# maetyu-d/audio-suite

Hardware: AMD Instinct MI355X
Metric: Msamples/sec rendered (microsound full pipe, 384 kHz->48 kHz) at 1/2/4/8 GPUs (higher is better)
Workload: dtype fp32; 1 GPU; C3: 384 kHz out, unfold x100 (30 MHz design SR), stretch x2, Poisson 18/s, 1 s, 16k-tap IR request (8192 cap), ER 320 taps, stereo; presets_per_gpu=1024, frames_per_gpu_step=393216000, sub_batches_per_gpu=3, parallelism=preset-sharded x1, streams_per_gpu=3, stream_gate=2,4, enqueue=threads

## Files before the change

audio-suite_amd/csrc/ctx.h:

```cpp
#pragma once
#include <atomic>
#include <cstdlib>
#include <cstring>
#include <map>
#include <memory>
#include <mutex>
#include <string>
#include <vector>

#include "dev_own.h"
#include "host_pool.h"

namespace {

std::mutex g_gate_mu;

struct Staging {
    struct Item { void** slot; const void* src; size_t bytes; };
    struct Slot { PinnedBuf host; Event done; bool armed = false; };
    Slot slot[2];
    int cur = 0;
    DevBuf<char> arena;
    std::vector<Item> items;
    template <class T> void add(T** dst, const T* src, size_t bytes) {
        items.push_back(Item{reinterpret_cast<void**>(dst), src, bytes});
    }
    hipError_t flush(hipStream_t s) {
        Slot& sl = slot[cur];
        hipError_t e = hipSuccess;
        if (!sl.done) e = sl.done.create(hipEventDisableTiming);
        if (e == hipSuccess && sl.armed) e = hipEventSynchronize(sl.done);
        std::vector<size_t> at(items.size());
        size_t total = 0;
        for (size_t i = 0; i < items.size(); ++i) {
            at[i] = total;
            total += (items[i].bytes + 255) & ~size_t(255);
        }
        total = std::max<size_t>(total, 256);
        if (e == hipSuccess && total > sl.host.cap) e = sl.host.alloc(total + total / 4 + 4096);
        if (e == hipSuccess && total > arena.cap) e = arena.alloc(total + total / 4 + 4096);
        if (e == hipSuccess) {
            constexpr size_t PIECE = size_t(1) << 20;
            std::vector<std::pair<size_t, size_t>> pieces;
// ... 17 lines not shown
    }
};

template <class T> struct Slice { T* p = nullptr; };

template <class P, class S>
struct PlanStoreT {
    std::vector<P> host;
    std::vector<DevBuf<S>> allocs;
    std::map<int, int> by_n;
    bool dirty = false;
    DevBuf<P> dev;
};
using PlanStore = PlanStoreT<RealPlan, float>;
using Plan64Store = PlanStoreT<Real64Plan, double>;

struct Switches {
    bool device_plan = false;
    bool fir4 = true;
    bool fir4c = true;
    bool fir8 = true;
    int fir64 = 1;
    int fir64_cap = FIR64_CAP;
    int fir8p = 1;
    bool fir8q = true;
    int fir8p_cus = 0;
    bool ola_fir = true;
    double ola_fir_density = 1.25;
    int h_early = 2;
    bool er_dev = true;
    int so_row = 0, so_col = 0;
    bool gen_share = true;
    bool spec_share = true;

    static Switches from_env() {
        Switches w;
        if (const char* e = getenv("MSGPU_DEVICE_PLAN")) w.device_plan = e[0] == '1';
        if (const char* e = getenv("MSGPU_FIR4")) w.fir4 = e[0] != '0';
        if (const char* e = getenv("MSGPU_FIR4C")) w.fir4c = e[0] != '0';
        if (const char* e = getenv("MSGPU_FIR8")) w.fir8 = e[0] != '0';
        if (const char* e = getenv("MSGPU_FIR64")) w.fir64 = atoi(e);
        if (const char* e = getenv("MSGPU_FIR64_CAP")) w.fir64_cap = std::max(1, std::min(FIR64_CAP, atoi(e)));
        if (const char* e = getenv("MSGPU_FIR8P")) w.fir8p = atoi(e);
        if (const char* e = getenv("MSGPU_FIR8Q")) w.fir8q = e[0] != '0';
        if (const char* e = getenv("MSGPU_FIR8P_CUS")) w.fir8p_cus = std::max(0, atoi(e));
        if (const char* e = getenv("MSGPU_OLA_FIR")) w.ola_fir = e[0] != '0';
        if (const char* e = getenv("MSGPU_OLA_FIR_DENSITY")) w.ola_fir_density = atof(e);
        if (const char* e = getenv("MSGPU_H_EARLY")) w.h_early = atoi(e);
        if (const char* e = getenv("MSGPU_ER_DEV")) w.er_dev = e[0] != '0';
        if (const char* e = getenv("MSGPU_SO_ROW")) w.so_row = atoi(e);
        if (const char* e = getenv("MSGPU_SO_COL")) w.so_col = atoi(e);
        if (const char* e = getenv("MSGPU_GEN_SHARE")) w.gen_share = e[0] != '0';
        if (const char* e = getenv("MSGPU_SPEC_SHARE")) w.spec_share = e[0] != '0';
        if (!w.gen_share) w.spec_share = false;        return w;
    }
};

struct Gate {
    msg_ctx* peer = nullptr;
    std::vector<msg_ctx*> gated_by;
    int wait = -1, rec = -1;
    Event ev;
    std::atomic<bool> armed{false};
};

struct Prof {
    bool on = false;
    int every = 1;
    int64_t n = 0;
    bool batch = false;
    Event ev[2][12];
    int cur = 0;
    bool pending[2] = {false, false};
    bool pending_fir[2] = {false, false};
    bool pending_h_early[2] = {false, false};
    double stage_sum[10] = {0};
    int64_t stage_cnt = 0;
    double host_sum[8] = {0};
    double ola_fir_sum = 0.0;
    double gen_events_sum = 0.0, gen_grains_sum = 0.0;
    double spec_runs_sum = 0.0;
    int64_t host_cnt = 0;

    hipError_t create_events() {
        for (auto& set : ev)
            for (Event& e : set)
                if (const hipError_t err = e.create()) return err;
// ... 171 lines not shown
```

audio-suite_amd/csrc/host_abi.inc:

```

int64_t msg_sizeof(int32_t which) {
    switch (which) {
        case 0: return (int64_t)sizeof(msg_preset);
        case 1: return (int64_t)sizeof(msg_event);
        case 2: return (int64_t)sizeof(msg_plan_info);
        case 3: return (int64_t)sizeof(msg_digest_rec);
        case 4: return (int64_t)sizeof(msg_loudness_rec);
        case 5: return (int64_t)sizeof(msg_truepeak_rec);
        case 6: return (int64_t)sizeof(msg_pcm_rec);
        case 7: return (int64_t)sizeof(msg_limit_rec);
        case 8: return (int64_t)sizeof(msg_lrange_rec);
        default: return -1;
    }
}

int msg_plan_host(const msg_preset* preset, const double* bp_bank, const double* ir_frag, int64_t ir_frag_len,
                  msg_plan_info* info, msg_event* events, int32_t max_events,
                  int32_t* er_off, double* er_gain) {
    (void)ir_frag;
    if (!preset || !info) return fail(nullptr, MSG_E_ARG, "null argument");
    for (int l = 0; l < 4; ++l)
        if (preset->n_bp[l] < 0 || (preset->n_bp[l] > 0 && (!bp_bank || preset->bp_off[l] < 0)))
            return fail(nullptr, MSG_E_ARG, "bad breakpoint lane");
    msg_plan_info sz;
// ... 225 lines not shown
            for (;;) {
                if (id == 0) {
                    for (;;) {
                        const double xx = -nprng::ZIG_NOR_INV_R * log1p(-nprng::next_double(g));
                        const double yy = -log1p(-nprng::next_double(g));
                        c += 2;
                        if (yy + yy > xx * xx) { v = ((ra >> 8) & 1) ? -(nprng::ZIG_NOR_R + xx) : nprng::ZIG_NOR_R + xx; break; }
                    }
                    break;
                }
                const double u = nprng::next_double(g);
                c += 1;
                if (((zig_fi_double[id - 1] - zig_fi_double[id]) * u + zig_fi_double[id]) < exp(-0.5 * xv * xv)) { v = xv; break; }
                uint64_t r = nprng::next_u64(g);
                c += 1;
                id = (int)(r & 0xff); r >>= 8;
                const int sign = (int)(r & 1);
                ra = (r >> 1) & 0x000fffffffffffffULL;
                xv = (double)ra * zig_wi_double[id];
                if (sign) xv = -xv;
                if (ra < zig_ki_double[id]) { v = xv; break; }
            }
            if (produced < n) out[produced] = v;
            ++produced;
            local = q + c;
        }
        do {
            for (int l = 0; l < 64; ++l) st[l] = j64.a * st[l] + g0.inc * j64.s;
            local -= 64;
        } while (local >= 64);
    }
    return MSG_OK;
}
```

audio-suite_amd/csrc/kernels_core.h:

```cpp
#pragma once
#include "rt.h"
#include "ola.h"
#include <type_traits>

__global__ void k_plan_sizes(const msg_preset* __restrict__ presets, int n_presets,
                             const double* __restrict__ bp, const int64_t* __restrict__ frag_len, nprng::Zig z,
                             msg_plan_info* __restrict__ info) {
    const int p = blockIdx.x * blockDim.x + threadIdx.x;
    if (p >= n_presets) return;
    msg_plan_info inf;
    msgplan::plan_sizes(presets[p], bp, z, frag_len[p], inf);
    info[p] = inf;
}

__global__ void k_plan_events(const msg_preset* __restrict__ presets, int n_presets,
                              const double* __restrict__ bp, const int64_t* __restrict__ frag_len, nprng::Zig z,
                              const int32_t* __restrict__ slot_base, const int32_t* __restrict__ tap_base,
                              msg_event* __restrict__ events, int32_t* __restrict__ er_off,
                              double* __restrict__ er_gain, msg_plan_info* __restrict__ info) {
    const int p = blockIdx.x * blockDim.x + threadIdx.x;
    if (p >= n_presets) return;
    msg_plan_info inf;
    const msg_preset& pr = presets[p];
    const bool er = (pr.flags & MSG_F_ER_CLOUD) != 0;
    msgplan::plan_events(pr, bp, z, frag_len[p], p, inf, events + slot_base[p],
                         er ? er_off + tap_base[p] : nullptr, er ? er_gain + tap_base[p] : nullptr);
    info[p] = inf;
}

#ifndef MSG_GEN_G
#define MSG_GEN_G 8
#endif
constexpr int GEN_G = MSG_GEN_G;
struct JumpTab {
    nprng::u128 a[GEN_T]; nprng::u128 s[GEN_T]; nprng::u128 a64, s64, aG, sG;
    uint2 kw[256]; float fif[256];
};

template <int G>
MSG_DEV int gen_walk(const uint64_t (&F)[G], const int (&consumed)[G], int local, uint32_t& vb, int& cnt) {
    cnt = 0;
    vb = 0;
#pragma unroll
    for (int g = 0; g < G; ++g) {
        if (local >= 64) { local -= 64; continue; }
        uint64_t valid = ~0ULL << local;
        uint64_t S = ~F[g] & valid;
        int pos = 64;
        while (S) {
            const int q = __builtin_ctzll(S);
            const int end = q + __builtin_amdgcn_readlane(consumed[g], q);
            const uint64_t after_q = ~((2ULL << q) - 1);
            const uint64_t before_end = end >= 64 ? ~0ULL : ((1ULL << end) - 1);
            valid &= ~(after_q & before_end);
            if (end >= 64) { pos = end; break; }
            S &= ~0ULL << end;
        }
        if (__builtin_amdgcn_inverse_ballot_w64(valid)) vb |= 1u << g;
        cnt += __popcll(valid);
        local = pos - 64;
    }
    return local;
}

MSG_DEV double slow_normal(nprng::u128 st, nprng::u128 inc, uint64_t rabs, int idx, double x,
                           const nprng::Zig& z, const uint64_t* ki, const double* wi, const float* fif,
                           int& consumed) {
    nprng::Pcg64 g;
    g.state = st; g.inc = inc; g.has_u32 = 0; g.u32 = 0;
// ... 62 lines not shown
    const float bv = h2 - hi;
    lo += (hi - (h2 - bv)) + (fl - bv);
    hi = h2;
    const float a = 2.0f * hi;
    const float sn = sinpif(a), cs = cospif(a);
    const float d = 6.2831853071795865f * lo;
    return make_float2(fmaf(d, cs, sn), fmaf(-d, sn, cs));
}
MSG_DEV float gen_basic_sample(const GenBasicConst& c, int j, float nrm) {
    float x;
    const float jf = (float)j;
    if (c.mode == MSG_GEN_RESONANT) {
        const float ph = ring_phase(jf, c.fa, c.fb);
        x = 0.9f * __builtin_amdgcn_sinf(ph) * __builtin_amdgcn_exp2f(fmaxf(jf * c.k_ring, -126.f)) +
            0.25f * nrm * __builtin_amdgcn_exp2f(fmaxf(jf * c.k_exc, -126.f));
    } else if (c.mode == MSG_GEN_GAUSSIAN_CLICK) {
        const float u = jf * c.inv_sigma;
        x = expf(-0.5f * (u * u)) * (nrm * 0.12f + 1.0f);
    } else if (c.mode == MSG_GEN_NOISE_BURST || c.mode == MSG_GEN_SKEWED) {
        return nrm;
    } else {
        x = nrm * 0.1f;
    }
    if (j < c.fade) x *= jf * c.inv_fade;
    if (j >= c.n - c.fade) x *= (float)(j - (c.n - c.fade)) * -c.inv_fade + 1.0f;
    return x;
}
MSG_DEV float gen_fade(const GenBasicConst& c, int j, float x) {
    if (j < c.fade) x *= (float)j * c.inv_fade;
    if (j >= c.n - c.fade) x *= (float)(j - (c.n - c.fade)) * -c.inv_fade + 1.0f;
    return x;
}

template <bool RAW64>
__global__ void __launch_bounds__(GEN_T)
k_gen_normal(const msg_preset* __restrict__ presets, const msg_event* __restrict__ events,
             const PresetRt* __restrict__ rt, const int32_t* __restrict__ ev_list, int n_list,
             nprng::Zig z, const JumpTab* __restrict__ jt, float* __restrict__ pool,
             double* __restrict__ pool64, const int64_t* __restrict__ off64) {
    __shared__ uint64_t s_ki[256];
    __shared__ double s_wi[256];
    __shared__ uint2 s_kw[256];
    __shared__ float s_fif[256];
    __shared__ float4 s_rot[128];
    __shared__ float4 s_base[64];
    const int li = blockIdx.x;
    if (li >= n_list) return;
    const int lane = (int)(threadIdx.x & (GEN_T - 1));
    for (int i = (int)threadIdx.x; i < 256; i += GEN_T) {
        s_ki[i] = z.ki[i];
        s_wi[i] = z.wi[i];
        s_kw[i] = jt->kw[i];
        s_fif[i] = jt->fif[i];
    }
    const msg_event& e = events[ev_list[li]];
    const msg_preset& pr = presets[e.preset];
    const PresetRt& r = rt[e.preset];
    const int n = e.n;
    float* out = pool + r.pool_base + e.pool_off;
    double* out64 = RAW64 ? pool64 + off64[li] : nullptr;

    GenBasicConst c;
    c.mode = pr.gen_mode == MSG_GEN_FALLBACK ? MSG_GEN_NOISE_BURST : pr.gen_mode;
    c.n = n;
    c.fade = (int)(0.01 * n) > 8 ? (int)(0.01 * n) : 8;
    c.inv_fade = (float)(1.0 / (double)c.fade);
    const double inv_sr = 1.0 / (double)e.gen_sr;
    const double f_over_sr = fmax(10.0, pr.ring_hz) * inv_sr;
    c.fa = (float)f_over_sr;
    c.fb = (float)(f_over_sr - (double)c.fa);
    const double log2e = 1.4426950408889634;
    c.k_ring = (float)(-inv_sr / fmax(1e-6, pr.ring_decay_ms / 1000.0) * log2e);
    c.k_exc = (float)(-inv_sr / fmax(1e-6, (pr.micro_ms / 1000.0) * 0.15) * log2e);
    const int sigma = (int)(0.0025 * n) > 1 ? (int)(0.0025 * n) : 1;
    c.inv_sigma = (float)(1.0 / (double)sigma);
    int q0 = -64;
    if (!RAW64 && c.mode == MSG_GEN_RESONANT) {
        for (int i = (int)threadIdx.x; i < 128; i += GEN_T) {
            const float rf = (float)i;
            const float2 sc = ring_sincos(rf, c.fa, c.fb);
            s_rot[i] = make_float4(sc.y, sc.x, 0.9f * __builtin_amdgcn_exp2f(rf * c.k_ring),
                                   0.25f * __builtin_amdgcn_exp2f(rf * c.k_exc));
        }
    }

    const nprng::Pcg64 g0 = nprng::default_rng((uint64_t)(pr.seed + e.index));
    const nprng::u128 inc = g0.inc;
    const nprng::u128 a64 = jt->a64;
    const nprng::u128 c64 = inc * jt->s64;

    constexpr int G = GEN_G;
    nprng::u128 st[G];
    st[0] = jt->a[lane] * g0.state + inc * jt->s[lane];
#pragma unroll
    for (int g = 1; g < G; ++g) st[g] = a64 * st[g - 1] + c64;
    const nprng::u128 aG = jt->aG;
    const nprng::u128 cG = inc * jt->sG;
    __syncthreads();

    int produced = 0;
    int local = 0;
    while (produced < n) {
        using XT = typename std::conditional<RAW64, double, float>::type;
        uint64_t rabs[G], F[G];
        int idx[G], consumed[G];
        (void)rabs; (void)idx;
        XT x[G];
        unsigned slow = 0;
#pragma unroll
        for (int g = 0; g < G; ++g) {
            consumed[g] = 1;
            bool fast;
            if constexpr (RAW64) {
                const uint64_t raw = nprng::xsl_rr(st[g]);
                const int id = (int)(raw & 0xff);
                const uint64_t rr = raw >> 8;
                rabs[g] = (rr >> 1) & 0x000fffffffffffffULL;
                idx[g] = id | (int)((rr & 1) << 8);
                x[g] = (double)rabs[g] * s_wi[id];
                if (rr & 1) x[g] = -x[g];
                fast = rabs[g] < s_ki[id];
            } else {
                const uint64_t hi = (uint64_t)(st[g] >> 64), lo = (uint64_t)st[g];
                const uint32_t rot = (uint32_t)(hi >> 58);
                uint32_t xl = (uint32_t)(hi ^ lo), xh = (uint32_t)((hi ^ lo) >> 32);
                if (rot & 32) { const uint32_t tmp = xl; xl = xh; xh = tmp; }
                const uint32_t olo = __builtin_amdgcn_alignbit(xh, xl, rot);
                const uint32_t ohi = __builtin_amdgcn_alignbit(xl, xh, rot);
                const uint32_t r32 = __builtin_amdgcn_alignbit(ohi, olo, 29);
                const int id = (int)(olo & 0xff);
                const uint2 kw = s_kw[id];
                const float xf = (float)r32 * __uint_as_float(kw.y);
                x[g] = (olo & 0x100) ? -xf : xf;
                fast = r32 < kw.x;
            }
            F[g] = __ballot(fast);
            if (!fast) slow |= 1u << g;
        }
        while (slow) {
            const int gs = __builtin_ctz(slow);
            slow &= slow - 1;
            nprng::u128 s0 = st[0];
#pragma unroll
            for (int g = 1; g < G; ++g)
                if (gs == g) s0 = st[g];
            const uint64_t raw = nprng::xsl_rr(s0);
            const int id = (int)(raw & 0xff);
            const uint64_t ra = (raw >> 9) & 0x000fffffffffffffULL;
            if (!RAW64 && ra < s_ki[id]) continue;
            double xv = (double)ra * s_wi[id];
            if ((raw >> 8) & 1) xv = -xv;
            int cn = 1;
            const double v = slow_normal(s0, inc, ra, id, xv, z, s_ki, s_wi, s_fif, cn);
#pragma unroll
            for (int g = 0; g < G; ++g)
                if (gs == g) { x[g] = (XT)v; consumed[g] = cn; }
        }
        uint32_t vb;
        int cnt;
        int pc = produced;
        local = gen_walk<G>(F, consumed, local, vb, cnt);
        produced += cnt;
        const bool reson = !RAW64 && c.mode == MSG_GEN_RESONANT;
#pragma unroll
        for (int g = 0; g < G; ++g) {
            const uint64_t valid = __ballot((vb >> g) & 1u);
            if (pc >= n || !valid) continue;
            if constexpr (RAW64) {
                if ((valid >> lane) & 1) {
                    const int j = pc + __popcll(valid & ((1ULL << lane) - 1));
                    if (j < n) out64[j] = x[g];
                }
            } else {
                const int rk = (int)__builtin_amdgcn_mbcnt_hi((uint32_t)(valid >> 32),
                                                              __builtin_amdgcn_mbcnt_lo((uint32_t)valid, 0u));
                const bool vl = __builtin_amdgcn_inverse_ballot_w64(valid);
                const int room = n - pc;
                float* __restrict__ ob = out + pc;
                if (reson) {
                    const int q = pc >> 6, d = pc & 63;
                    if (q - q0 >= 64) {
                        q0 = q;
                        const float jb = (float)(64 * (q0 + lane));
                        const float2 sc = ring_sincos(jb, c.fa, c.fb);
                        __syncthreads();
                        s_base[lane] = make_float4(sc.x, sc.y, __builtin_amdgcn_exp2f(fmaxf(jb * c.k_ring, -126.f)),
                                                   __builtin_amdgcn_exp2f(fmaxf(jb * c.k_exc, -126.f)));
                        __syncthreads();
                    }
                    const float4 u = s_base[q - q0];
                    const bool edge = pc < c.fade || pc + 64 > c.n - c.fade;
                    if (vl && rk < room) {
                        const float4 tb = s_rot[rk + d];
                        float v = fmaf(u.x, tb.x, u.y * tb.y) * (u.z * tb.z) + x[g] * (u.w * tb.w);
                        if (edge) v = gen_fade(c, pc + rk, v);
                        ob[rk] = v;
                    }
                } else if (vl && rk < room) {
                    ob[rk] = gen_basic_sample(c, pc + rk, (float)x[g]);
                }
            }
            pc += __popcll(valid);
        }
#pragma unroll
        for (int g = 0; g < G; ++g) st[g] = aG * st[g] + cG;
    }
}

constexpr int ER_T = 256;

MSG_DEV double er_uniform(nprng::Pcg64& g, double lo, double hi) {
    return __dadd_rn(lo, __dmul_rn(hi - lo, nprng::next_double(g)));
}

__global__ void __launch_bounds__(ER_T)
k_er_gains(const msg_preset* __restrict__ presets, const PresetRt* __restrict__ rt, int n_presets,
           const int32_t* __restrict__ er_key, const int32_t* __restrict__ er_first,
           const int32_t* __restrict__ er_cnt, double* __restrict__ g_tap, double* __restrict__ er_gain) {
    const int p = blockIdx.x;
    if (p >= n_presets) return;
    const msg_preset& pr = presets[p];
    if (!(pr.flags & MSG_F_ER_CLOUD)) return;
    const PresetRt& r = rt[p];
// ... 109 lines not shown
```

audio-suite_amd/csrc/msgpu.hip:

```cpp
#include <hip/hip_runtime.h>
#include <algorithm>
#include <cmath>
#include <cstdio>
#include <cstring>
#include <deque>
#include <map>
#include <sched.h>
#include <atomic>
#include <chrono>
#include <condition_variable>
#include <functional>
#include <memory>
#include <mutex>
#include <optional>
#include <string>
#include <thread>
#include <vector>

#include "msg_common.h"
#include "ziggurat_tables.h"
#include "nprng.h"
#include "plan.h"
#include "fftplan.h"
#include "fft_lds.h"
// ... 295 lines not shown
}

template <class T>
static int sf_upload(msg_ctx* ctx, hipStream_t s, const std::vector<PresetRt>& prt, const std::vector<int2>& jobs,
                     const int64_t* irjobs, size_t n_irjobs, DevBuf<T>& taps_dev, const T* taps, int64_t M) {
    HIPCHK(ctx, ctx->sf_prt.ensure(prt.size()));
    HIPCHK(ctx, ctx->sf_jobs.ensure(jobs.size()));
    HIPCHK(ctx, taps_dev.ensure((size_t)M));
    HIPCHK(ctx, ctx->sf_irjobs.ensure(n_irjobs));
    HIPCHK(ctx, hipMemcpyAsync(ctx->sf_prt.p, prt.data(), sizeof(PresetRt) * prt.size(), hipMemcpyHostToDevice, s));
    HIPCHK(ctx, hipMemcpyAsync(ctx->sf_jobs.p, jobs.data(), sizeof(int2) * jobs.size(), hipMemcpyHostToDevice, s));
    HIPCHK(ctx, hipMemcpyAsync(taps_dev.p, taps, sizeof(T) * (size_t)M, hipMemcpyHostToDevice, s));
    HIPCHK(ctx, hipMemcpyAsync(ctx->sf_irjobs.p, irjobs, sizeof(int64_t) * n_irjobs, hipMemcpyHostToDevice, s));
    return MSG_OK;
}

extern "C" {

int msg_abi_version(void) { return MSG_ABI_VERSION; }

int msg_host_threads(void) { return HostPool::get().threads(); }

const char* msg_last_error(msg_ctx* ctx) { return ctx ? ctx->err.c_str() : g_err.c_str(); }

msg_ctx* msg_create(int device_ordinal) {
    int ndev = 0;
    hipError_t e = hipGetDeviceCount(&ndev);
    if (e != hipSuccess || ndev <= 0) { g_err = "no HIP device available"; return nullptr; }
    if (device_ordinal < 0 || device_ordinal >= ndev) { g_err = "bad device ordinal"; return nullptr; }
    if (hipSetDevice(device_ordinal) != hipSuccess) { g_err = "hipSetDevice failed"; return nullptr; }
    std::unique_ptr<msg_ctx> ctx(new msg_ctx());
    ctx->device = device_ordinal;
    ctx->sw = Switches::from_env();
    auto up = [](auto& dst, const auto* src, size_t n) { return dst.upload(src, n) == hipSuccess; };
    auto up2 = [](DevBuf<float2>& dst, bool ok, const std::vector<float>& tab) {
        return ok && dst.upload(reinterpret_cast<const float2*>(tab.data()), tab.size() / 2) == hipSuccess;
    };
    if (!up(ctx->d_ki, zig_ki_double, 256) || !up(ctx->d_wi, zig_wi_double, 256) ||
        !up(ctx->d_fi, zig_fi_double, 256) || !up(ctx->d_ke, zig_ke_double, 256) ||
        !up(ctx->d_we, zig_we_double, 256) || !up(ctx->d_fe, zig_fe_double, 256)) {
        g_err = "uploading ziggurat tables failed";
        return nullptr;
    }
    ctx->dzig = nprng::Zig{ctx->d_ki.p, ctx->d_wi.p, ctx->d_fi.p, ctx->d_ke.p, ctx->d_we.p, ctx->d_fe.p};
    JumpTab jt;
    for (int l = 0; l < GEN_T; ++l) {
        const nprng::Jump j = nprng::jump_of((uint64_t)l + 1);
        jt.a[l] = j.a; jt.s[l] = j.s;
    }
    const nprng::Jump j64 = nprng::jump_of(GEN_T);
    jt.a64 = j64.a; jt.s64 = j64.s;
    const nprng::Jump jG = nprng::jump_of((uint64_t)GEN_T * GEN_G);
    jt.aG = jG.a; jt.sG = jG.s;
    for (int i = 0; i < 256; ++i) {
        const float w = (float)(zig_wi_double[i] * 1048576.0);
        uint32_t wb;
        memcpy(&wb, &w, 4);
        jt.kw[i] = make_uint2((uint32_t)(zig_ki_double[i] >> 20), wb);
        jt.fif[i] = (float)zig_fi_double[i];
    }
    if (!up(ctx->d_jump, &jt, 1)) { g_err = "uploading jump table failed"; return nullptr; }
    std::vector<float> tab;
    for (int i = 0; i < 5; ++i)
        if (!up2(ctx->d_fir2tab[i], fir2_tables_host(1024 << i, tab), tab)) {
            g_err = "uploading FIR twiddle tables failed";
            return nullptr;
        }
    if (!up2(ctx->d_fir4tab, fir4_tables_host(16384, tab), tab)) {
        g_err = "uploading FIR4 twiddle tables failed";
        return nullptr;
    }
    for (int i = 0; i < SPEC_CT_PLANS; ++i)
        if (!up2(ctx->d_spec_ct_tab[i], spectral_ct_tables(i, tab), tab)) {
            g_err = "uploading spectral twiddle tables failed";
            return nullptr;
        }
    if (!up2(ctx->d_spec3_tab, spec3_tables(tab), tab)) {
        g_err = "uploading spectral twiddle tables failed";
        return nullptr;
    }
    {
        float tp_tab[TP_TAB_N];
        tp_table(tp_tab);
        if (!up(ctx->d_tp_tab, tp_tab, (size_t)TP_TAB_N)) { g_err = "uploading the true-peak taps failed"; return nullptr; }
    }
    int cu = 0;
// ... 391 lines not shown
```

audio-suite_amd/csrc/render_stages.h:

```cpp
#pragma once

static int stage_check(msg_ctx* ctx, Batch& b) {
    for (int p = 0; p < b.P; ++p) {
        for (int l = 0; l < 4; ++l) {
            const int32_t nb = b.presets[p].n_bp[l], ob = b.presets[p].bp_off[l];
            if (nb < 0 || (nb > 0 && (!b.bp_bank || ob < 0 || (int64_t)ob + nb > b.bp_pairs)))
                return fail(ctx, MSG_E_ARG, "preset " + std::to_string(p) + ": breakpoint lane outside the bank");
        }
        const int ic = b.presets[p].ir_conv;
        if (ic >= b.n_irs || (ic >= 0 && !b.irs)) return fail(ctx, MSG_E_ARG, "bad IR index");
    }
    return MSG_OK;
}

static int plan_bases(msg_ctx* ctx, Batch& b) {
    b.nslots = b.ntaps = 0;
    int64_t frames = 0;
    for (int p = 0; p < b.P; ++p) {
        b.slot_base[p] = (int32_t)b.nslots;
        b.tap_base[p] = (int32_t)b.ntaps;
        b.nslots += b.info[p].n_slots;
        if (b.presets[p].flags & MSG_F_ER_CLOUD) b.ntaps += std::max(1, b.presets[p].er_taps);
        if (b.info[p].out_n > MSG_MAX_FRAMES) return fail(ctx, MSG_E_UNSUPPORTED, "output longer than 2^31 - 2^20 frames");
        frames += b.info[p].out_n;
// ... 752 lines not shown
static int enqueue_h_spectra(msg_ctx* ctx, Batch& b) {
    const Batch::Fir& F = b.fir;
    hipStream_t s = b.s;
    const double* erg = er_gains(ctx, b);
    if (b.er_dev && b.ntaps > 0) {
        hipLaunchKernelGGL(k_er_gains, dim3((unsigned)b.P), dim3(ER_T), 0, s, ctx->presets.p, ctx->prt.p, b.P,
                           ctx->er_key.p, ctx->er_first.p, ctx->er_cnt.p, ctx->er_tap_d.p, ctx->er_gain_d.p);
        HIPCHK(ctx, hipGetLastError());
    }
    if (F.htiles > 0)
        HIPCHK(ctx, launch_h_build((unsigned)F.htiles, s, ctx->prt.p, ctx->h_tile_begin.p, b.P, ctx->er_off.p,
                                   erg, ctx->irbank.p, ctx->hscratch.p));
    if (!F.ir8.jobs.empty())
        HIPCHK(ctx, launch_fir8_spec64((unsigned)(F.ir8.jobs.size() / 4), s, ctx->ir8_jobs.p, ctx->d_fir4tab.p,
                                       ctx->irbank.p, ctx->hspec.p));
    if (!F.hpart_jobs.empty())
        HIPCHK(ctx, launch_fir4_hpart(16384, (unsigned)F.hpart_jobs.size(), s, ctx->prt.p, ctx->hpart_jobs.p,
                                      ctx->d_fir4tab.p, ctx->hscratch.p, ctx->hspec.p));
    if (!F.ir8.er_list.empty())
        HIPCHK(ctx, launch_fir8_hconv((unsigned)F.ir8.er_list.size(), s, ctx->prt.p, ctx->fir8_list.p, ctx->d_fir4tab.p,
                                      ctx->er_off.p, erg, ctx->hspec.p));
    if (!F.ir4.jobs.empty())
        HIPCHK(ctx, launch_fir4_irspec((unsigned)(F.ir4.jobs.size() / 4), s, ctx->ir4_jobs.p, ctx->d_fir4tab.p,
                                       ctx->irbank.p, ctx->hspec.p));
    if (!F.ir4.er_list.empty())
        HIPCHK(ctx, launch_fir4_hconv((unsigned)F.ir4.er_list.size(), s, ctx->prt.p, ctx->fir4c_list.p, ctx->d_fir4tab.p,
                                      ctx->er_off.p, erg, ctx->hspec.p));
    if (F.hblocks_gen > 0)
        HIPCHK(ctx, launch_fir_h((unsigned)F.hblocks, F.lds, s, ctx->prt.p, ctx->h_begin.p, b.P,
                                 ctx->fir_plans.dev.p, ctx->fir_plan_of.p, ctx->hscratch.p, ctx->hspec.p));
    return MSG_OK;
}

static int enqueue_generate(msg_ctx* ctx, Batch& b) {
    const std::vector<int32_t>& gen = b.f32.gen_list;
    const std::vector<int32_t>& gen64 = b.g64.gen_list;
    if (!gen.empty())
        hipLaunchKernelGGL(k_gen_normal<false>, dim3((unsigned)gen.size()), dim3(GEN_T), 0, b.s,
                           ctx->presets.p, ctx->events.p, ctx->prt.p, ctx->gen_list.p, (int)gen.size(),
                           ctx->dzig, ctx->d_jump.p, ctx->micro.p, (double*)nullptr, (const int64_t*)nullptr);
    HIPCHK(ctx, hipGetLastError());
    if (!gen64.empty())
        hipLaunchKernelGGL(k_gen_normal<true>, dim3((unsigned)gen64.size()), dim3(GEN_T), 0, b.s,
                           ctx->presets.p, ctx->events.p, ctx->prt.p, ctx->gen64_list.p, (int)gen64.size(),
                           ctx->dzig, ctx->d_jump.p, ctx->micro.p, ctx->micro64.p, (const int64_t*)ctx->gen64_off.p);
    HIPCHK(ctx, hipGetLastError());
    return MSG_OK;
}

static int enqueue_spectral(msg_ctx* ctx, Batch& b) {
    const Batch::F32& F = b.f32;
    const Batch::G64& G = b.g64;
    hipStream_t s = b.s;
    if (!F.spec3.empty())
        HIPCHK(ctx, launch_spec3((unsigned)F.spec3.size(), s, ctx->events.p, ctx->ert.p, ctx->prt.p, ctx->d_spec3_tab.p,
                                 ctx->spec3_list.p, (int)F.spec3.size(), ctx->micro.p, ctx->grain.p));
    for (int i = 0; i < SPEC_CT_PLANS; ++i)
        if (F.ct_off[i + 1] > F.ct_off[i])
            HIPCHK(ctx, launch_spectral_ct(i, (unsigned)(F.ct_off[i + 1] - F.ct_off[i]), s, ctx->events.p, ctx->ert.p,
                                           ctx->prt.p, ctx->d_spec_ct_tab[i].p, ctx->spec_ct_list.p + F.ct_off[i],
                                           F.ct_off[i + 1] - F.ct_off[i], ctx->micro.p, ctx->grain.p));
    if (!F.spec_small.empty())
        HIPCHK(ctx, launch_spectral(false, (unsigned)F.spec_small.size(), F.small_lds, s, ctx->presets.p,
                                    ctx->events.p, ctx->ert.p, ctx->prt.p, ctx->grain_plans.dev.p, ctx->spec_small.p,
                                    (int)F.spec_small.size(), ctx->micro.p, ctx->grain.p));
    if (!F.spec_big.empty())
        HIPCHK(ctx, launch_spectral(true, (unsigned)F.spec_big.size(), F.big_lds, s, ctx->presets.p,
                                    ctx->events.p, ctx->ert.p, ctx->prt.p, ctx->grain_plans.dev.p, ctx->spec_big.p,
                                    (int)F.spec_big.size(), ctx->micro.p, ctx->grain.p));
    if (!G.lds.empty())
        HIPCHK(ctx, launch_grain64(nullptr, (unsigned)G.lds.size(), G.cap * 16, s, ctx->presets.p, ctx->ev64.p,
                                   ctx->prt.p, ctx->plans64.dev.p, ctx->g64_list.p, (int)G.lds.size(),
                                   ctx->irbank.p, ctx->imgbank.p, ctx->dzig, ctx->micro64.p, ctx->grain64.p,
                                   ctx->save64.p, ctx->grain.p));
    if (!G.glb.empty())
        HIPCHK(ctx, launch_grain64(&G.gg, G.g_grid, 0, s, ctx->presets.p, ctx->ev64.p, ctx->prt.p, ctx->plans64.dev.p,
                                   ctx->g64_list.p + G.lds.size(), (int)G.glb.size(), ctx->irbank.p,
                                   ctx->imgbank.p, ctx->dzig, ctx->micro64.p, ctx->grain64.p, ctx->save64.p,
// ... 184 lines not shown
```

audio-suite_amd/msgpu/_lib.py:

```python
from __future__ import annotations

import ctypes as C
import os
import threading

HERE = os.path.dirname(os.path.abspath(__file__))
LIB_PATH = os.environ.get("MSGPU_LIB") or os.path.join(HERE, "libmsgpu.so")
ABI_VERSION = 2

MSG_OK, MSG_E_VALUE, MSG_E_UNSUPPORTED, MSG_E_DEVICE, MSG_E_ARG = 0, 1, 2, 3, 4

SPEC_ROUTES = ("copy", "small", "big", "ct37500", "ct30000", "ct2400", "ct1920", "ct1500", "ct480", "spec3", "f64")

GEN_MODE = {"Gaussian click": 0, "Dust impulses": 1, "Noise burst": 2, "Skewed transient": 3,
            "Resonant strike": 4, "Crackle / corona": 5, "Stick–slip friction": 6,
            "Micro-chaos": 7, "Wavelet atoms": 8, "IR fragment": 9, "Image scanline": 10}
GEN_FALLBACK = 11
PROCESS = {"Single": 0, "Poisson": 1, "Clustered": 2, "Hawkes": 3}
PROC_NONE = 4
F_STEREO, F_BANDLIMIT, F_PARTIAL_LOCK, F_NL_WARP, F_CEP_WARP, F_GRAIN_OFFSET = (1 << i for i in range(6))
F_RES_BANK, F_WAVEGUIDE, F_EVENT_FEEDBACK, F_IMPRINT, F_ER_CLOUD, F_SPACE_IR, F_MULTIBAND = \
    (1 << i for i in range(6, 13))


# ... 116 lines not shown
    "msg_loudness": (C.c_int, [C.c_void_p, C.c_void_p, C.c_int32, C.POINTER(C.c_int64), C.POINTER(C.c_int64), C.c_int32,
                               C.c_int32, C.c_void_p, C.c_void_p]),
    "msg_loudness_range": (C.c_int, [C.c_void_p, C.c_void_p, C.c_int32, C.POINTER(C.c_int64), C.POINTER(C.c_int64),
                                     C.c_int32, C.c_int32, C.c_void_p, C.c_void_p, C.c_void_p, C.POINTER(C.c_int64),
                                     C.c_void_p]),
    "msg_lrange_hops_host": (C.c_int, [C.c_void_p, C.c_int64, C.c_int64, C.c_void_p]),
    "msg_loudness_range_host": (C.c_int, [C.c_void_p, C.c_int32, C.c_int64, C.c_int32, C.c_void_p, C.c_void_p]),
    "msg_loudness_gain": (C.c_int, [C.c_void_p, C.c_void_p, C.c_int32, C.POINTER(C.c_int64), C.POINTER(C.c_int64),
                                    C.c_int32, C.c_void_p, C.c_double, C.c_double, C.c_void_p]),
    "msg_loudness_host": (C.c_int, [C.c_void_p, C.c_int32, C.c_int64, C.c_int32, C.c_void_p]),
    "msg_truepeak": (C.c_int, [C.c_void_p, C.c_void_p, C.c_int32, C.POINTER(C.c_int64), C.POINTER(C.c_int64), C.c_int32,
                               C.c_int32, C.c_void_p, C.c_void_p]),
    "msg_truepeak_gain": (C.c_int, [C.c_void_p, C.c_void_p, C.c_int32, C.POINTER(C.c_int64), C.POINTER(C.c_int64),
                                    C.c_int32, C.c_void_p, C.c_void_p, C.c_double, C.c_double, C.c_double, C.c_void_p]),
    "msg_truepeak_host": (C.c_int, [C.c_void_p, C.c_int32, C.c_int64, C.c_int32, C.c_void_p]),
    "msg_quantize": (C.c_int, [C.c_void_p, C.c_void_p, C.c_int32, C.POINTER(C.c_int64), C.POINTER(C.c_int64), C.c_int32,
                               C.c_int32, C.c_int32, C.c_uint64, C.POINTER(C.c_uint64), C.c_void_p,
                               C.POINTER(C.c_int64), C.c_void_p, C.c_void_p]),
    "msg_quantize_host": (C.c_int, [C.c_void_p, C.c_int32, C.c_int64, C.c_int32, C.c_int32, C.c_uint64, C.c_uint64,
                                    C.c_void_p, C.c_void_p]),
    "msg_quantize_shaped": (C.c_int, [C.c_void_p, C.c_void_p, C.c_int32, C.POINTER(C.c_int64), C.POINTER(C.c_int64),
                                      C.c_int32, C.c_int32, C.c_int32, C.c_int32, C.c_uint64, C.POINTER(C.c_uint64),
                                      C.c_void_p, C.POINTER(C.c_int64), C.c_void_p, C.c_void_p]),
    "msg_quantize_shaped_host": (C.c_int, [C.c_void_p, C.c_int32, C.c_int64, C.c_int32, C.c_int32, C.c_int32, C.c_uint64,
                                           C.c_uint64, C.c_void_p, C.c_void_p]),
    "msg_limit": (C.c_int, [C.c_void_p, C.c_void_p, C.c_int32, C.POINTER(C.c_int64), C.POINTER(C.c_int64), C.c_int32,
                            C.c_int32, C.c_double, C.c_int32, C.c_void_p, C.c_void_p, C.c_void_p]),
    "msg_limit_host": (C.c_int, [C.c_void_p, C.c_int32, C.c_int64, C.c_int32, C.c_double, C.c_int32, C.c_void_p]),
    "msg_rng_raw": (C.c_int, [C.c_uint64, C.POINTER(C.c_uint64), C.c_int64]),
    "msg_rng_normal": (C.c_int, [C.c_uint64, C.POINTER(C.c_double), C.c_int64]),
    "msg_rng_exponential": (C.c_int, [C.c_uint64, C.POINTER(C.c_double), C.c_int64]),
    "msg_rng_integers": (C.c_int, [C.c_uint64, C.c_int64, C.c_int64, C.POINTER(C.c_int64), C.c_int64]),
    "msg_rng_normal_chunked": (C.c_int, [C.c_uint64, C.POINTER(C.c_double), C.c_int64]),
}
EXPORTS = tuple(_PROTOS)

_lib = None
_lock = threading.Lock()


def lib() -> C.CDLL:
    global _lib
    with _lock:
        if _lib is None:
            if not os.path.exists(LIB_PATH):
                raise RuntimeError(f"libmsgpu not built: {LIB_PATH} is missing "
                                   "(run `python -c 'import __graft_entry__ as g; g.build()'`)")
            if os.environ.get("MSGPU_HOST_ONLY") != "1":
                try:
                    import torch
                except ImportError:
                    pass
            L = C.CDLL(LIB_PATH)
            for name, (res, args) in _PROTOS.items():
                f = getattr(L, name)
                f.restype = res
                f.argtypes = args
            if L.msg_abi_version() != ABI_VERSION:
                raise RuntimeError("libmsgpu ABI version mismatch")
            for which, st in enumerate((MsgPreset, MsgEvent, MsgPlanInfo, MsgDigestRec, MsgLoudnessRec,
                                        MsgTruePeakRec, MsgPcmRec, MsgLimitRec, MsgLRangeRec)):
                if L.msg_sizeof(which) != C.sizeof(st):
                    raise RuntimeError(f"libmsgpu struct {st.__name__} size mismatch: "
                                       f"{L.msg_sizeof(which)} != {C.sizeof(st)}")
            _lib = L
    return _lib
# ... 12 lines not shown
```

include/msgpu.h:

```cpp
#ifndef MSGPU_H
#define MSGPU_H

#include <stddef.h>
#include <stdint.h>

#ifdef __cplusplus
extern "C" {
#endif

#define MSG_ABI_VERSION 2

enum msg_gen_mode {
    MSG_GEN_GAUSSIAN_CLICK = 0, MSG_GEN_DUST = 1, MSG_GEN_NOISE_BURST = 2,
    MSG_GEN_SKEWED = 3, MSG_GEN_RESONANT = 4, MSG_GEN_CRACKLE = 5,
    MSG_GEN_STICK_SLIP = 6, MSG_GEN_MICRO_CHAOS = 7, MSG_GEN_WAVELET = 8,
    MSG_GEN_IR_FRAGMENT = 9, MSG_GEN_IMAGE = 10,
    MSG_GEN_FALLBACK = 11
};
enum msg_process { MSG_PROC_SINGLE = 0, MSG_PROC_POISSON = 1, MSG_PROC_CLUSTERED = 2,
                   MSG_PROC_HAWKES = 3, MSG_PROC_NONE = 4 };
enum msg_flag {
    MSG_F_STEREO = 1u << 0, MSG_F_BANDLIMIT = 1u << 1, MSG_F_PARTIAL_LOCK = 1u << 2,
    MSG_F_NL_WARP = 1u << 3, MSG_F_CEP_WARP = 1u << 4, MSG_F_GRAIN_OFFSET = 1u << 5,
    MSG_F_RES_BANK = 1u << 6, MSG_F_WAVEGUIDE = 1u << 7, MSG_F_EVENT_FEEDBACK = 1u << 8,
// ... 151 lines not shown
    int32_t q_min, q_max;
    int32_t bits, dither;
} msg_pcm_rec;
int msg_quantize(msg_ctx* ctx, const float* x_dev, int32_t channels, const int64_t* offsets, const int64_t* n,
                 int32_t n_signals, int32_t bits, int32_t dither, uint64_t seed, const uint64_t* keys,
                 void* out_dev, const int64_t* out_byte_off, msg_pcm_rec* rec_dev, void* stream);
int msg_quantize_host(const float* x, int32_t channels, int64_t n, int32_t bits, int32_t dither, uint64_t seed,
                      uint64_t key, void* out, msg_pcm_rec* rec);

enum msg_shape { MSG_SHAPE_E3 = 1, MSG_SHAPE_LIPSHITZ5 = 2, MSG_SHAPE_F9 = 3 };
int msg_quantize_shaped(msg_ctx* ctx, const float* x_dev, int32_t channels, const int64_t* offsets, const int64_t* n,
                        int32_t n_signals, int32_t bits, int32_t dither, int32_t shape, uint64_t seed,
                        const uint64_t* keys, void* out_dev, const int64_t* out_byte_off, msg_pcm_rec* rec_dev,
                        void* stream);
int msg_quantize_shaped_host(const float* x, int32_t channels, int64_t n, int32_t bits, int32_t dither, int32_t shape,
                             uint64_t seed, uint64_t key, void* out, msg_pcm_rec* rec);

typedef struct msg_limit_rec {
    double min_gain, reduction_db;
    int64_t limited_frames;
    int32_t lookahead, state;
} msg_limit_rec;
int msg_limit(msg_ctx* ctx, float* x_dev, int32_t channels, const int64_t* offsets, const int64_t* n,
              int32_t n_signals, int32_t sr, double ceiling_tp, int32_t lookahead_frames,
              const msg_truepeak_rec* tp_rec_dev, msg_limit_rec* rec_dev, void* stream);
int msg_limit_host(float* x, int32_t channels, int64_t n, int32_t sr, double ceiling_tp,
                   int32_t lookahead_frames, msg_limit_rec* rec);

int msg_rng_raw(uint64_t seed, uint64_t* out, int64_t n);
int msg_rng_normal(uint64_t seed, double* out, int64_t n);
int msg_rng_exponential(uint64_t seed, double* out, int64_t n);
int msg_rng_integers(uint64_t seed, int64_t low, int64_t high, int64_t* out, int64_t n);
int msg_rng_normal_chunked(uint64_t seed, double* out, int64_t n);

#ifdef __cplusplus
}
#endif
#endif
```

Measured before the change: 88580 Msamples/s.

## Split each event's normal generation across K cooperating waves

The normal-noise generator kernel now launches K waves per event. Each wave jumps the PCG stream to its own 512-draw group, classifies its draws independently, and then the waves stitch their ziggurat carry-over offsets in order through shared memory, re-walking only when a group's carry is nonzero. A host rule picks K from list length, event length and CU count so that short lists of long events fill the GPU, and MSGPU_GEN_K can override it. The cost is extra block barriers per round and larger blocks. Host reference functions are added to check the wave-split ordering.

```diff
diff --git a/audio-suite_amd/csrc/ctx.h b/audio-suite_amd/csrc/ctx.h
--- a/audio-suite_amd/csrc/ctx.h
+++ b/audio-suite_amd/csrc/ctx.h
@@ -9,6 +9,7 @@
 #include <vector>
 
 #include "dev_own.h"
+#include "gen_waves.h"
 #include "host_pool.h"
 
 namespace {
@@ -92,6 +93,7 @@
     int so_row = 0, so_col = 0;
     bool gen_share = true;
     bool spec_share = true;
+    int gen_k = 0;
 
     static Switches from_env() {
         Switches w;
@@ -112,7 +114,9 @@
         if (const char* e = getenv("MSGPU_SO_COL")) w.so_col = atoi(e);
         if (const char* e = getenv("MSGPU_GEN_SHARE")) w.gen_share = e[0] != '0';
         if (const char* e = getenv("MSGPU_SPEC_SHARE")) w.spec_share = e[0] != '0';
-        if (!w.gen_share) w.spec_share = false;        return w;
+        if (const char* e = getenv("MSGPU_GEN_K")) w.gen_k = (e[0] >= '0' && e[0] <= '9') ? atoi(e) : -1;
+        if (!w.gen_share) w.spec_share = false;
+        return w;
     }
 };
 
diff --git a/audio-suite_amd/csrc/gen_waves.h b/audio-suite_amd/csrc/gen_waves.h
--- /dev/null
+++ b/audio-suite_amd/csrc/gen_waves.h
@@ -0,0 +1,26 @@
+#pragma once
+#include <cstdint>
+
+namespace genwaves {
+
+constexpr int KMAX = 16;
+constexpr int GROUP = 512;
+constexpr int WAVES_PER_CU = 16;
+constexpr int LONG_LIST_PER_CU = 8;
+constexpr int SHARED_K = 4;
+constexpr int SMALL_LIST_PER_CU_INV = 4;
+
+inline bool valid_k(int k) { return k == 1 || k == 2 || k == 4 || k == 8 || k == 16; }
+
+inline int gen_waves(int64_t list_len, int64_t n_max, int n_cu) {
+    if (list_len <= 0 || n_max <= GROUP || n_cu <= 0) return 1;
+    if (list_len >= (int64_t)LONG_LIST_PER_CU * n_cu) return 1;
+    const int64_t groups = (n_max + GROUP - 1) / GROUP;
+    const int64_t room = (int64_t)WAVES_PER_CU * n_cu / list_len;
+    const int kmax = list_len * SMALL_LIST_PER_CU_INV <= n_cu ? KMAX : SHARED_K;
+    int k = 1;
+    while (2 * k <= kmax && 2 * k <= groups && 2 * k <= room) k *= 2;
+    return k;
+}
+
+}
diff --git a/audio-suite_amd/csrc/host_abi.inc b/audio-suite_amd/csrc/host_abi.inc
--- a/audio-suite_amd/csrc/host_abi.inc
+++ b/audio-suite_amd/csrc/host_abi.inc
@@ -281,3 +281,123 @@
     }
     return MSG_OK;
 }
+
+namespace {
+constexpr int KW_GROUP = 512;
+struct KwGroup {
+    double x[KW_GROUP];
+    int consumed[KW_GROUP];
+    int cnt = 0, over = 0;
+    int first = 0;
+};
+void kw_classify(nprng::u128 st, nprng::u128 inc, const nprng::Jump& j1, KwGroup& G) {
+    for (int l = 0; l < KW_GROUP; ++l) {
+        st = j1.a * st + inc * j1.s;
+        const uint64_t raw = nprng::xsl_rr(st);
+        int id = (int)(raw & 0xff);
+        const uint64_t rr = raw >> 8;
+        uint64_t ra = (rr >> 1) & 0x000fffffffffffffULL;
+        double xv = (double)ra * zig_wi_double[id];
+        if (rr & 1) xv = -xv;
+        G.x[l] = xv;
+        G.consumed[l] = 1;
+        if (ra < zig_ki_double[id]) continue;
+        nprng::Pcg64 g;
+        g.state = st; g.inc = inc; g.has_u32 = 0; g.u32 = 0;
+        int c = 1;
+        double v = 0.0;
+        for (;;) {
+            if (id == 0) {
+                for (;;) {
+                    const double xx = -nprng::ZIG_NOR_INV_R * log1p(-nprng::next_double(g));
+                    const double yy = -log1p(-nprng::next_double(g));
+                    c += 2;
+                    if (yy + yy > xx * xx) { v = ((ra >> 8) & 1) ? -(nprng::ZIG_NOR_R + xx) : nprng::ZIG_NOR_R + xx; break; }
+                }
+                break;
+            }
+            const double u = nprng::next_double(g);
+            c += 1;
+            if (((zig_fi_double[id - 1] - zig_fi_double[id]) * u + zig_fi_double[id]) < exp(-0.5 * xv * xv)) { v = xv; break; }
+            uint64_t r = nprng::next_u64(g);
+            c += 1;
+            id = (int)(r & 0xff); r >>= 8;
+            const int sign = (int)(r & 1);
+            ra = (r >> 1) & 0x000fffffffffffffULL;
+            xv = (double)ra * zig_wi_double[id];
+            if (sign) xv = -xv;
+            if (ra < zig_ki_double[id]) { v = xv; break; }
+        }
+        G.x[l] = v;
+        G.consumed[l] = c;
+    }
+}
+void kw_walk(KwGroup& G, int local) {
+    G.first = local;
+    G.cnt = 0;
+    int p = local;
+    while (p < KW_GROUP) { p += G.consumed[p]; ++G.cnt; }
+    G.over = p - KW_GROUP;
+}
+void kw_emit(const KwGroup& G, int64_t pw, double* out, int64_t n) {
+    int64_t j = pw;
+    for (int p = G.first; p < KW_GROUP && j < n; p += G.consumed[p]) out[j++] = G.x[p];
+}
+}
+
+int msg_rng_normal_kwaves(uint64_t seed, int32_t K, double* out, int64_t n, int64_t* rewalks) {
+    if (!(K == 1 || K == 2 || K == 4 || K == 8 || K == 16)) return fail(nullptr, MSG_E_VALUE, "K must be 1, 2, 4, 8 or 16");
+    if (n < 0 || (n > 0 && !out)) return fail(nullptr, MSG_E_VALUE, "bad output");
+    const nprng::Pcg64 g0 = nprng::default_rng(seed);
+    const nprng::Jump j1 = nprng::jump_of(1);
+    const nprng::Jump jR = nprng::jump_of((uint64_t)KW_GROUP * (uint64_t)K);
+    std::vector<KwGroup> grp((size_t)K);
+    std::vector<nprng::u128> st((size_t)K);
+    for (int w = 0; w < K; ++w) st[w] = nprng::apply_jump(nprng::jump_of((uint64_t)KW_GROUP * (uint64_t)w), g0.state, g0.inc);
+    int64_t produced = 0, rw = 0;
+    int local = 0;
+    while (produced < n) {
+        for (int w = 0; w < K; ++w) {
+            kw_classify(st[w], g0.inc, j1, grp[w]);
+            kw_walk(grp[w], 0);
+        }
+        int lin = local;
+        for (int j = 0; j < K; ++j) {
+            if (lin != 0) {
+                if (lin >= KW_GROUP) { grp[j].first = KW_GROUP; grp[j].cnt = 0; grp[j].over = lin - KW_GROUP; }
+                else kw_walk(grp[j], lin);
+                ++rw;
+            }
+            kw_emit(grp[j], produced, out, n);
+            produced += grp[j].cnt;
+            lin = grp[j].over;
+        }
+        local = lin;
+        for (int w = 0; w < K; ++w) st[w] = jR.a * st[w] + g0.inc * jR.s;
+    }
+    if (rewalks) *rewalks = rw;
+    return MSG_OK;
+}
+
+int64_t msg_rng_normal_carries(uint64_t seed, int64_t n, int32_t* carry, int64_t max_groups) {
+    if (n < 0 || max_groups < 0 || (max_groups > 0 && !carry)) return -1;
+    const nprng::Pcg64 g0 = nprng::default_rng(seed);
+    const nprng::Jump j1 = nprng::jump_of(1);
+    const nprng::Jump jG = nprng::jump_of((uint64_t)KW_GROUP);
+    std::vector<KwGroup> Gv(1);
+    KwGroup* const G = Gv.data();
+    nprng::u128 st = g0.state;
+    int64_t produced = 0, groups = 0;
+    int local = 0;
+    while (produced < n) {
+        if (groups < max_groups) carry[groups] = local;
+        kw_classify(st, g0.inc, j1, *G);
+        if (local >= KW_GROUP) { G->cnt = 0; G->over = local - KW_GROUP; }
+        else kw_walk(*G, local);
+        produced += G->cnt;
+        local = G->over;
+        st = jG.a * st + g0.inc * jG.s;
+        ++groups;
+    }
+    return groups;
+}
diff --git a/audio-suite_amd/csrc/kernels_core.h b/audio-suite_amd/csrc/kernels_core.h
--- a/audio-suite_amd/csrc/kernels_core.h
+++ b/audio-suite_amd/csrc/kernels_core.h
@@ -32,9 +32,13 @@
 #define MSG_GEN_G 8
 #endif
 constexpr int GEN_G = MSG_GEN_G;
+constexpr int GEN_KMAX = 16;
+MSG_HD constexpr int gen_k_log2(int k) { return k <= 1 ? 0 : 1 + gen_k_log2(k / 2); }
 struct JumpTab {
     nprng::u128 a[GEN_T]; nprng::u128 s[GEN_T]; nprng::u128 a64, s64, aG, sG;
     uint2 kw[256]; float fif[256];
+    nprng::u128 aW[GEN_KMAX], sW[GEN_KMAX];
+    nprng::u128 aR[4], sR[4];
 };
 
 template <int G>
@@ -163,8 +167,8 @@
     return x;
 }
 
-template <bool RAW64>
-__global__ void __launch_bounds__(GEN_T)
+template <bool RAW64, int K>
+__global__ void __launch_bounds__(GEN_T * K)
 k_gen_normal(const msg_preset* __restrict__ presets, const msg_event* __restrict__ events,
              const PresetRt* __restrict__ rt, const int32_t* __restrict__ ev_list, int n_list,
              nprng::Zig z, const JumpTab* __restrict__ jt, float* __restrict__ pool,
@@ -174,11 +178,17 @@
     __shared__ uint2 s_kw[256];
     __shared__ float s_fif[256];
     __shared__ float4 s_rot[128];
-    __shared__ float4 s_base[64];
+    __shared__ float4 s_base[K * 64];
+    __shared__ int2 s_carry[2][K];
+    static_assert(K == 1 || K == 2 || K == 4 || K == 8 || K == GEN_KMAX, "waves per event");
+    (void)s_carry;
     const int li = blockIdx.x;
     if (li >= n_list) return;
     const int lane = (int)(threadIdx.x & (GEN_T - 1));
-    for (int i = (int)threadIdx.x; i < 256; i += GEN_T) {
+    int wv = 0;
+    if constexpr (K > 1) wv = __builtin_amdgcn_readfirstlane((int)(threadIdx.x / GEN_T));
+    float4* const sb = s_base + 64 * wv;
+    for (int i = (int)threadIdx.x; i < 256; i += GEN_T * K) {
         s_ki[i] = z.ki[i];
         s_wi[i] = z.wi[i];
         s_kw[i] = jt->kw[i];
@@ -207,7 +217,7 @@
     c.inv_sigma = (float)(1.0 / (double)sigma);
     int q0 = -64;
     if (!RAW64 && c.mode == MSG_GEN_RESONANT) {
-        for (int i = (int)threadIdx.x; i < 128; i += GEN_T) {
+        for (int i = (int)threadIdx.x; i < 128; i += GEN_T * K) {
             const float rf = (float)i;
             const float2 sc = ring_sincos(rf, c.fa, c.fb);
             s_rot[i] = make_float4(sc.y, sc.x, 0.9f * __builtin_amdgcn_exp2f(rf * c.k_ring),
@@ -223,14 +233,18 @@
     constexpr int G = GEN_G;
     nprng::u128 st[G];
     st[0] = jt->a[lane] * g0.state + inc * jt->s[lane];
+    if constexpr (K > 1) st[0] = jt->aW[wv] * st[0] + inc * jt->sW[wv];
 #pragma unroll
     for (int g = 1; g < G; ++g) st[g] = a64 * st[g - 1] + c64;
-    const nprng::u128 aG = jt->aG;
-    const nprng::u128 cG = inc * jt->sG;
+    constexpr int KL = gen_k_log2(K);
+    const nprng::u128 aG = K > 1 ? jt->aR[K > 1 ? KL - 1 : 0] : jt->aG;
+    const nprng::u128 cG = inc * (K > 1 ? jt->sR[K > 1 ? KL - 1 : 0] : jt->sG);
     __syncthreads();
 
     int produced = 0;
     int local = 0;
+    int rpar = 0;
+    (void)rpar;
     while (produced < n) {
         using XT = typename std::conditional<RAW64, double, float>::type;
         uint64_t rabs[G], F[G];
@@ -290,18 +304,45 @@
         uint32_t vb;
         int cnt;
         int pc = produced;
-        local = gen_walk<G>(F, consumed, local, vb, cnt);
-        produced += cnt;
+        if constexpr (K == 1) {
+            local = gen_walk<G>(F, consumed, local, vb, cnt);
+            produced += cnt;
+        } else {
+            int lout = gen_walk<G>(F, consumed, 0, vb, cnt);
+            if (lane == 0) s_carry[rpar][wv] = make_int2(cnt, lout);
+            __syncthreads();
+            int lin = local;
+#pragma unroll 1
+            for (int j = 0; j < K; ++j) {
+                if (__builtin_expect(lin != 0, 0)) {
+                    if (wv == j) {
+                        lout = gen_walk<G>(F, consumed, lin, vb, cnt);
+                        if (lane == 0) s_carry[rpar][j] = make_int2(cnt, lout);
+                    }
+                    __syncthreads();
+                }
+                const int2 cj = s_carry[rpar][j];
+                if (wv == j) pc = produced;
+                produced += __builtin_amdgcn_readfirstlane(cj.x);
+                lin = __builtin_amdgcn_readfirstlane(cj.y);
+            }
+            local = lin;
+            rpar ^= 1;
+        }
         const bool reson = !RAW64 && c.mode == MSG_GEN_RESONANT;
 #pragma unroll
         for (int g = 0; g < G; ++g) {
             const uint64_t valid = __ballot((vb >> g) & 1u);
             if (pc >= n || !valid) continue;
-            if constexpr (RAW64) {
+            if constexpr (RAW64 && K == 1) {
                 if ((valid >> lane) & 1) {
                     const int j = pc + __popcll(valid & ((1ULL << lane) - 1));
                     if (j < n) out64[j] = x[g];
                 }
+            } else if constexpr (RAW64) {
+                const int rk = (int)__builtin_amdgcn_mbcnt_hi((uint32_t)(valid >> 32),
+                                                              __builtin_amdgcn_mbcnt_lo((uint32_t)valid, 0u));
+                if (__builtin_amdgcn_inverse_ballot_w64(valid) && rk < n - pc) out64[pc + rk] = x[g];
             } else {
                 const int rk = (int)__builtin_amdgcn_mbcnt_hi((uint32_t)(valid >> 32),
                                                               __builtin_amdgcn_mbcnt_lo((uint32_t)valid, 0u));
@@ -314,12 +355,22 @@
                         q0 = q;
                         const float jb = (float)(64 * (q0 + lane));
                         const float2 sc = ring_sincos(jb, c.fa, c.fb);
-                        __syncthreads();
-                        s_base[lane] = make_float4(sc.x, sc.y, __builtin_amdgcn_exp2f(fmaxf(jb * c.k_ring, -126.f)),
-                                                   __builtin_amdgcn_exp2f(fmaxf(jb * c.k_exc, -126.f)));
-                        __syncthreads();
+                        if constexpr (K == 1) {
+                            __syncthreads();
+                        } else {
+                            __builtin_amdgcn_fence(__ATOMIC_ACQ_REL, "wavefront");
+                            __builtin_amdgcn_wave_barrier();
+                        }
+                        sb[lane] = make_float4(sc.x, sc.y, __builtin_amdgcn_exp2f(fmaxf(jb * c.k_ring, -126.f)),
+                                               __builtin_amdgcn_exp2f(fmaxf(jb * c.k_exc, -126.f)));
+                        if constexpr (K == 1) {
+                            __syncthreads();
+                        } else {
+                            __builtin_amdgcn_fence(__ATOMIC_ACQ_REL, "wavefront");
+                            __builtin_amdgcn_wave_barrier();
+                        }
                     }
-                    const float4 u = s_base[q - q0];
+                    const float4 u = sb[q - q0];
                     const bool edge = pc < c.fade || pc + 64 > c.n - c.fade;
                     if (vl && rk < room) {
                         const float4 tb = s_rot[rk + d];
diff --git a/audio-suite_amd/csrc/msgpu.hip b/audio-suite_amd/csrc/msgpu.hip
--- a/audio-suite_amd/csrc/msgpu.hip
+++ b/audio-suite_amd/csrc/msgpu.hip
@@ -351,6 +351,10 @@
     std::unique_ptr<msg_ctx> ctx(new msg_ctx());
     ctx->device = device_ordinal;
     ctx->sw = Switches::from_env();
+    if (ctx->sw.gen_k != 0 && !genwaves::valid_k(ctx->sw.gen_k)) {
+        g_err = "MSGPU_GEN_K must be 0 (the rule), 1, 2, 4, 8 or 16";
+        return nullptr;
+    }
     auto up = [](auto& dst, const auto* src, size_t n) { return dst.upload(src, n) == hipSuccess; };
     auto up2 = [](DevBuf<float2>& dst, bool ok, const std::vector<float>& tab) {
         return ok && dst.upload(reinterpret_cast<const float2*>(tab.data()), tab.size() / 2) == hipSuccess;
@@ -371,6 +375,14 @@
     jt.a64 = j64.a; jt.s64 = j64.s;
     const nprng::Jump jG = nprng::jump_of((uint64_t)GEN_T * GEN_G);
     jt.aG = jG.a; jt.sG = jG.s;
+    for (int w = 0; w < GEN_KMAX; ++w) {
+        const nprng::Jump jw = nprng::jump_of((uint64_t)GEN_T * GEN_G * w);
+        jt.aW[w] = jw.a; jt.sW[w] = jw.s;
+    }
+    for (int i = 0; i < 4; ++i) {
+        const nprng::Jump jr = nprng::jump_of((uint64_t)GEN_T * GEN_G * (2u << i));
+        jt.aR[i] = jr.a; jt.sR[i] = jr.s;
+    }
     for (int i = 0; i < 256; ++i) {
         const float w = (float)(zig_wi_double[i] * 1048576.0);
         uint32_t wb;
diff --git a/audio-suite_amd/csrc/render_stages.h b/audio-suite_amd/csrc/render_stages.h
--- a/audio-suite_amd/csrc/render_stages.h
+++ b/audio-suite_amd/csrc/render_stages.h
@@ -808,18 +808,38 @@
     return MSG_OK;
 }
 
+template <bool RAW64>
+static void launch_gen(msg_ctx* ctx, Batch& b, const std::vector<int32_t>& list, const int32_t* d_list,
+                       double* pool64, const int64_t* off64) {
+    int k = ctx->sw.gen_k;
+    if (k == 0) {
+        int n_max = 0;
+        for (int32_t ei : list) n_max = std::max(n_max, (int)ctx->h_events[ei].n);
+        k = genwaves::gen_waves((int64_t)list.size(), n_max, ctx->n_cu);
+    }
+    const dim3 grid((unsigned)list.size());
+    const int n_list = (int)list.size();
+#define MSG_GEN_LAUNCH(K)                                                                                    \
+    hipLaunchKernelGGL((k_gen_normal<RAW64, K>), grid, dim3(GEN_T * K), 0, b.s, ctx->presets.p, ctx->events.p, \
+                       ctx->prt.p, d_list, n_list, ctx->dzig, ctx->d_jump.p, ctx->micro.p, pool64, off64)
+    switch (k) {
+    case 2: MSG_GEN_LAUNCH(2); break;
+    case 4: MSG_GEN_LAUNCH(4); break;
+    case 8: MSG_GEN_LAUNCH(8); break;
+    case 16: MSG_GEN_LAUNCH(16); break;
+    default: MSG_GEN_LAUNCH(1); break;
+    }
+#undef MSG_GEN_LAUNCH
+}
+
 static int enqueue_generate(msg_ctx* ctx, Batch& b) {
     const std::vector<int32_t>& gen = b.f32.gen_list;
     const std::vector<int32_t>& gen64 = b.g64.gen_list;
     if (!gen.empty())
-        hipLaunchKernelGGL(k_gen_normal<false>, dim3((unsigned)gen.size()), dim3(GEN_T), 0, b.s,
-                           ctx->presets.p, ctx->events.p, ctx->prt.p, ctx->gen_list.p, (int)gen.size(),
-                           ctx->dzig, ctx->d_jump.p, ctx->micro.p, (double*)nullptr, (const int64_t*)nullptr);
+        launch_gen<false>(ctx, b, gen, ctx->gen_list.p, (double*)nullptr, (const int64_t*)nullptr);
     HIPCHK(ctx, hipGetLastError());
     if (!gen64.empty())
-        hipLaunchKernelGGL(k_gen_normal<true>, dim3((unsigned)gen64.size()), dim3(GEN_T), 0, b.s,
-                           ctx->presets.p, ctx->events.p, ctx->prt.p, ctx->gen64_list.p, (int)gen64.size(),
-                           ctx->dzig, ctx->d_jump.p, ctx->micro.p, ctx->micro64.p, (const int64_t*)ctx->gen64_off.p);
+        launch_gen<true>(ctx, b, gen64, ctx->gen64_list.p, ctx->micro64.p, (const int64_t*)ctx->gen64_off.p);
     HIPCHK(ctx, hipGetLastError());
     return MSG_OK;
 }
diff --git a/audio-suite_amd/msgpu/_lib.py b/audio-suite_amd/msgpu/_lib.py
--- a/audio-suite_amd/msgpu/_lib.py
+++ b/audio-suite_amd/msgpu/_lib.py
@@ -172,6 +172,8 @@
     "msg_rng_exponential": (C.c_int, [C.c_uint64, C.POINTER(C.c_double), C.c_int64]),
     "msg_rng_integers": (C.c_int, [C.c_uint64, C.c_int64, C.c_int64, C.POINTER(C.c_int64), C.c_int64]),
     "msg_rng_normal_chunked": (C.c_int, [C.c_uint64, C.POINTER(C.c_double), C.c_int64]),
+    "msg_rng_normal_kwaves": (C.c_int, [C.c_uint64, C.c_int32, C.POINTER(C.c_double), C.c_int64, C.POINTER(C.c_int64)]),
+    "msg_rng_normal_carries": (C.c_int64, [C.c_uint64, C.c_int64, C.POINTER(C.c_int32), C.c_int64]),
 }
 EXPORTS = tuple(_PROTOS)
 
diff --git a/include/msgpu.h b/include/msgpu.h
--- a/include/msgpu.h
+++ b/include/msgpu.h
@@ -207,6 +207,8 @@
 int msg_rng_exponential(uint64_t seed, double* out, int64_t n);
 int msg_rng_integers(uint64_t seed, int64_t low, int64_t high, int64_t* out, int64_t n);
 int msg_rng_normal_chunked(uint64_t seed, double* out, int64_t n);
+int msg_rng_normal_kwaves(uint64_t seed, int32_t K, double* out, int64_t n, int64_t* rewalks);
+int64_t msg_rng_normal_carries(uint64_t seed, int64_t n, int32_t* carry, int64_t max_groups);
 
 #ifdef __cplusplus
 }
```

After: 89800 Msamples/s (median of 6 runs). +1.4%, better.
